# NVIDIA-Genomics-Research/DL4VC

Hardware: AMD Instinct MI355X
Metric: candidate-variants/sec (DAN fwd, 64 reads x 201 bp) (higher is better)
Workload: dtype f32

## Files before the change

dl4vc_amd/csrc/dan_device.h:

```cpp
#pragma once
#include "dan_kernels.h"

namespace dan {

typedef float v4f __attribute__((ext_vector_type(4)));

__device__ __forceinline__ v4f mfma16(float a, float b, v4f c) {
    return __builtin_amdgcn_mfma_f32_16x16x4f32(a, b, c, 0, 0, 0);
}

__device__ __forceinline__ v4f splat(float x) { return (v4f){x, x, x, x}; }

typedef const __attribute__((address_space(1))) v4f* gv4f_ptr;

__device__ __forceinline__ float relu1(float v) { return __builtin_amdgcn_fmed3f(v, 0.f, __builtin_inff()); }

__device__ __forceinline__ void gemm_tile(v4f (&acc)[NT], const v4f (&a)[NT], v4f& b, const float* next) {
#pragma unroll
    for (int s = 0; s < 4; ++s)
#pragma unroll
        for (int n = 0; n < NT; ++n) acc[n] = mfma16(a[n][s], b[s], acc[n]);
    b = *(const v4f*)next;
}

__device__ __forceinline__ void conv_gemm(v4f (&acc)[MTW][NT], const float* xs, gv4f_ptr wl, const v4f (&a_first)[NT],
                                          int kg, int ntaps, int dil, int lane, int m_base, int cnt) {
    const int pos = lane & 15, kk = lane >> 4;
    const int total = ntaps * kg;
    const int t0 = (ntaps == 3) ? -dil : 0;
    const float* xrow = xs + (HALO + m_base * 16 + pos) * LDS_S + kk * 4;
    const bool full = cnt == MTW;
    v4f a_nxt[NT], b[MTW];
#pragma unroll
    for (int n = 0; n < NT; ++n) a_nxt[n] = a_first[n];
    {
        const float* xb = xrow + t0 * LDS_S;
#pragma unroll
        for (int m = 0; m < MTW - 1; ++m) b[m] = *(const v4f*)(xb + m * 16 * LDS_S);
        b[MTW - 1] = full ? *(const v4f*)(xb + (MTW - 1) * 16 * LDS_S) : splat(0.f);
    }
    int t = 0, g = 0;
    for (int it = 0; it < total; ++it) {
        v4f a[NT];
#pragma unroll
        for (int n = 0; n < NT; ++n) a[n] = a_nxt[n];
        const int nx = (it + 1 < total) ? it + 1 : it;
#pragma unroll
        for (int n = 0; n < NT; ++n) a_nxt[n] = wl[(size_t)nx * (KGC * 64) + n * 64];
        int tn = t, gn = g + 1;
        if (gn == kg) { gn = 0; ++tn; }
        if (it + 1 == total) { tn = t; gn = g; }
        const float* xn = xrow + (t0 + tn * dil) * LDS_S + gn * 16;
#pragma unroll
        for (int m = 0; m < MTW - 1; ++m) gemm_tile(acc[m], a, b[m], xn + m * 16 * LDS_S);
        __builtin_amdgcn_sched_group_barrier(0x020, NT, 0);
#pragma unroll
        for (int m = 0; m < MTW - 1; ++m) {
            __builtin_amdgcn_sched_group_barrier(0x008, 4 * NT, 0);
            __builtin_amdgcn_sched_group_barrier(0x100, 1, 0);
        }
        if (full) gemm_tile(acc[MTW - 1], a, b[MTW - 1], xn + (MTW - 1) * 16 * LDS_S);
        t = tn; g = gn;
    }
}

template <int NW, bool RANGE = false, int TILES = MT>
__device__ __forceinline__ void bottleneck(const float* xs, const v4f (&wf)[KGC], const float* bbot, float* hrow, int L,
                                           int wave, int lane, int p_lo = 0) {
    constexpr int PSTEP = NW / 2;
    constexpr int NBT = (TILES + PSTEP - 1) / PSTEP;
    lane = (int)__builtin_amdgcn_mbcnt_hi(~0u, __builtin_amdgcn_mbcnt_lo(~0u, 0u));
    asm volatile("" : "+v"(lane));
    const int pos = lane & 15, kk = lane >> 4;
    const int n = wave & 1, p0 = wave >> 1;
    const float* xrow = xs + (HALO + pos) * LDS_S + kk * 4;
    int roff[NBT];
#pragma unroll
    for (int i = 0; i < NBT; ++i) roff[i] = min(p0 + PSTEP * i, TILES - 1) * 16 * LDS_S;
    v4f acc[NBT], b[NBT];
    {
        const v4f bias = *(const v4f*)(bbot + n * 16 + kk * 4);
#pragma unroll
        for (int i = 0; i < NBT; ++i) acc[i] = bias;
    }
#pragma unroll
    for (int i = 0; i < NBT; ++i) b[i] = *(const v4f*)(xrow + roff[i]);
#pragma unroll
    for (int g = 0; g < KGC; ++g) {
        const int gn = (g + 1 < KGC) ? g + 1 : g;
#pragma unroll
        for (int i = 0; i < NBT; ++i) {
#pragma unroll
            for (int s = 0; s < 4; ++s) acc[i] = mfma16(wf[g][s], b[i][s], acc[i]);
            b[i] = *(const v4f*)(xrow + roff[i] + gn * 16);
        }
#pragma unroll
        for (int i = 0; i < NBT; ++i) {
            __builtin_amdgcn_sched_group_barrier(0x008, 4, 0);
            __builtin_amdgcn_sched_group_barrier(0x100, 1, 0);
        }
    }
#pragma unroll
    for (int i = 0; i < NBT; ++i) {
        const int pt = p0 + PSTEP * i, p = pt * 16 + pos;
        if (pt < TILES && p < L && (!RANGE || p >= p_lo)) {
            v4f v = acc[i];
#pragma unroll
            for (int j = 0; j < 4; ++j) v[j] = relu1(v[j]);
            *(v4f*)((char*)hrow + (unsigned)(p * HPAD + n * 16 + kk * 4) * 4u) = v;
        }
    }
}

__device__ __forceinline__ void copy_out(const float* xs, float* dst, int lo, int hi, int tid) {
    for (int i = lo * (CPAD / 4) + tid; i < hi * (CPAD / 4); i += SEG_THREADS) {
        const int p = i >> 5, c4 = i & 31;
        ((v4f*)dst)[i] = *(const v4f*)(xs + (HALO + p) * LDS_S + c4 * 4);
    }
}

constexpr int MW = 7;
constexpr int WHB = 102;
constexpr int MW_SHORT = 6;
constexpr int WHB_SHORT = 94;
constexpr int MPOS_SHORT = WHB_SHORT + 16 * MW_SHORT;
constexpr int wino_half_base(int tw) { return tw == MW ? WHB : WHB_SHORT; }
constexpr int wino_cover(int tw) { return tw == MW ? MPOS : MPOS_SHORT; }
template <int TW = MW>
__device__ __forceinline__ int wino_base(int lane) {
    const int n = lane & 15;
    const int c = n & 1, hf = (n >> 2) & 1, q = ((n >> 1) & 1) + 2 * (((n >> 3) ^ (n >> 2)) & 1);
    return hf * wino_half_base(TW) + 4 * q * TW + c;
}

typedef float v2f __attribute__((ext_vector_type(2)));
__device__ __forceinline__ v4f pk_sub(v4f a, v4f b, v2f m1) {
    const v2f lo = __builtin_elementwise_fma((v2f){b[0], b[1]}, m1, (v2f){a[0], a[1]});
    const v2f hi = __builtin_elementwise_fma((v2f){b[2], b[3]}, m1, (v2f){a[2], a[3]});
    return (v4f){lo[0], lo[1], hi[0], hi[1]};
}
__device__ __forceinline__ v4f pk_add(v4f a, v4f b) { return a + b; }
template <int TW>
__device__ __forceinline__ void conv_gemm_wino(v4f (&acc)[TW][4], const float* xrow, gv4f_ptr wl, const v4f (&a_first)[4]) {
    v4f a_nxt[4];
#pragma unroll
    for (int k = 0; k < 4; ++k) a_nxt[k] = a_first[k];
    v4f xa = *(const v4f*)(xrow), xb = *(const v4f*)(xrow + 2 * LDS_S), xc = *(const v4f*)(xrow + 4 * LDS_S),
        xd = *(const v4f*)(xrow + 6 * LDS_S);
    float neg1 = -1.f;
    asm volatile("" : "+v"(neg1));
    const v2f m1 = {neg1, neg1};
    for (int g = 0; g < KGC; ++g) {
        v4f a[4];
#pragma unroll
        for (int k = 0; k < 4; ++k) a[k] = a_nxt[k];
        const int gn = (g + 1 < KGC) ? g + 1 : g;
#pragma unroll
        for (int k = 0; k < 4; ++k) a_nxt[k] = wl[(size_t)(k * KGC + gn) * (KGC * 64)];
        const float* xg = xrow + g * 16;
        const float* xn = xrow + gn * 16;
#pragma unroll
        for (int m = 0; m < TW; ++m) {
            v4f v[4];
            v[0] = pk_sub(xa, xc, m1); v[1] = pk_add(xb, xc); v[2] = pk_sub(xc, xb, m1); v[3] = pk_sub(xb, xd, m1);
            if (m + 1 < TW) {
                xa = xc; xb = xd;
                xc = *(const v4f*)(xg + (4 * m + 8) * LDS_S);
                xd = *(const v4f*)(xg + (4 * m + 10) * LDS_S);
            } else {
                xa = *(const v4f*)(xn); xb = *(const v4f*)(xn + 2 * LDS_S);
                xc = *(const v4f*)(xn + 4 * LDS_S); xd = *(const v4f*)(xn + 6 * LDS_S);
            }
            __builtin_amdgcn_s_setprio(3);
#pragma unroll
            for (int s = 0; s < 4; ++s)
#pragma unroll
                for (int k = 0; k < 4; ++k) acc[m][k] = mfma16(a[k][s], v[k][s], acc[m][k]);
            __builtin_amdgcn_s_setprio(0);
        }
    }
}

constexpr int WINO_ROWS_READ = HALO + WHB + 4 * (4 * MW - 1) + 1 + 4 + 1;

}
```

dl4vc_amd/csrc/dan_kernels.hip:

```cpp
#include "dan_device.h"

namespace dan {

#ifdef DAN_STAMPS
__device__ unsigned long long* g_stamps;
constexpr int NSTAMP = 64;
#define STAMP(k)                                                                                      \
    do {                                                                                              \
        __builtin_amdgcn_sched_barrier(0);                                                            \
        unsigned long long t_ = __builtin_amdgcn_s_memtime();                                         \
        __builtin_amdgcn_s_waitcnt(0xC07F);                                                           \
        if (lane == 0 && (k) < NSTAMP) g_stamps[((size_t)stamp_row * NWAVE + wave) * NSTAMP + (k)] = t_; \
        __builtin_amdgcn_sched_barrier(0);                                                            \
    } while (0)
#else
#define STAMP(k) do {} while (0)
#endif

static_assert((HALO + WHB + 4 * (4 * MW - 1) + 1 + 4 + 1) * LDS_S <= LDS_ROWS * LDS_S + MAX_LAYERS * CST_FLOATS, "wino reads stay inside LDS");
static_assert(WHB + 4 * (4 * MW - 1) + 3 >= MPOS - 1 && 4 * (4 * MW - 1) + 3 >= WHB - 1, "wino tiling covers the read");
static_assert(WHB_SHORT + 4 * (4 * MW_SHORT - 1) + 3 >= MPOS_SHORT - 1 && 4 * (4 * MW_SHORT - 1) + 3 >= WHB_SHORT - 1 && WHB_SHORT % 4 == 2,
              "short wino tiling covers its unit");

template <int TW>
__device__ __forceinline__ void gemm1x1_wino(v4f (&acc)[TW][2], const float* xrow, gv4f_ptr wl, v4f a_first) {
    v4f a_nxt = a_first, b[TW][2];
#pragma unroll
    for (int m = 0; m < TW; ++m)
#pragma unroll
        for (int o = 0; o < 2; ++o) b[m][o] = *(const v4f*)(xrow + (4 * m + 2 * o) * LDS_S);
    for (int g = 0; g < KGC; ++g) {
        const v4f a = a_nxt;
        const int gn = (g + 1 < KGC) ? g + 1 : g;
        a_nxt = wl[(size_t)gn * (KGC * 64)];
#pragma unroll
        for (int m = 0; m < TW; ++m) {
            __builtin_amdgcn_s_setprio(3);
#pragma unroll
            for (int s = 0; s < 4; ++s)
#pragma unroll
                for (int o = 0; o < 2; ++o) acc[m][o] = mfma16(a[s], b[m][o][s], acc[m][o]);
            __builtin_amdgcn_s_setprio(0);
#pragma unroll
            for (int o = 0; o < 2; ++o) b[m][o] = *(const v4f*)(xrow + (4 * m + 2 * o) * LDS_S + gn * 16);
        }
    }
}

template <bool WINO, bool PERSIST, bool SPLIT, int TW = MW, bool FOLD = false>
__global__ __launch_bounds__(SEG_THREADS, NWAVE / 4) void segment_kernel(SegmentArgs a_by_value) {
    static_assert(!FOLD || (PERSIST && !SPLIT), "the site-owning form is a persistent one-unit form");
    static_assert((!(SPLIT && WINO) && TW == MW) || (SPLIT && WINO && TW == MW_SHORT), "six tiles per lane: the split Winograd kernel, and only it");
    constexpr int TILES = TW == MW ? MT : (MPOS_SHORT + 15) / 16;
    __shared__ __attribute__((aligned(16))) float lds[LDS_ROWS * LDS_S + MAX_LAYERS * CST_FLOATS];
    float* const xs = lds;
    float* const cst = lds + LDS_ROWS * LDS_S;
    typedef const __attribute__((address_space(4))) SegmentArgs* kernarg_ptr;
    constexpr int UNITS = SPLIT ? 2 : 1;
    const int n_work = FOLD ? a_by_value.n_sites : (a_by_value.work_count ? *a_by_value.work_count : a_by_value.n_rows) * UNITS;
    const int per = FOLD ? a_by_value.xcd_sites : a_by_value.work_count ? (n_work + 7) >> 3 : a_by_value.xcd_rows * UNITS;
    const int xcd = blockIdx.x & 7;
    int j = blockIdx.x >> 3;
    int wk = xcd * per + j;
    if (j >= per || wk >= n_work) return;
    [[maybe_unused]] int fold_r = 0;
next_row:
    {
    kernarg_ptr ap = (kernarg_ptr)__builtin_amdgcn_kernarg_segment_ptr();
    if (PERSIST) asm volatile("" : "+s"(ap));
    auto args = [&]() -> decltype(auto) { if constexpr (PERSIST) return (*ap); else return (a_by_value); };
    const auto& a = args();
    [[maybe_unused]] const int unit = wk & 1;
    const int L = SPLIT ? (unit ? a.u_len[1] : a.u_len[0]) : a.L;
    const int Lw = SPLIT ? a.Lw : L;
    const int u_off = SPLIT ? (unit ? a.u_off[1] : a.u_off[0]) : 0;
    [[maybe_unused]] const int own_lo = SPLIT ? (unit ? a.own_lo[1] : a.own_lo[0]) : 0;
    [[maybe_unused]] const int own_hi = SPLIT ? (unit ? a.own_hi[1] : a.own_hi[0]) : L;
    [[maybe_unused]] const int stamp_row = wk;
    int tid = threadIdx.x;
    if (PERSIST) asm volatile("" : "+v"(tid));
    const int lane = tid & 63;
    const int wave = __builtin_amdgcn_readfirstlane(tid >> 6);
    const int wrow = SPLIT ? wk >> 1 : wk;
    const int row_index = FOLD ? wk * a.R + fold_r : __builtin_amdgcn_readfirstlane(a.work_count ? a.work[wrow] : wrow);
    const int site = FOLD ? wk : (int)((unsigned)row_index / (unsigned)a.R);
    const int r = FOLD ? fold_r : row_index - site * a.R;
    const size_t read_idx = (size_t)site * a.R + r;
    float* yrow = a.y + (read_idx * (size_t)Lw + u_off) * CPAD;
    float* yout = SPLIT ? a.y_out + (read_idx * (size_t)Lw + u_off) * CPAD : yrow;
    const int pos = lane & 15, kk = lane >> 4;
    const int cq = wave & 3, ph = wave >> 2;
    const int m_base = ph * MTW, cnt = ph ? MT - MTW : MTW;
    int chb[NT];
#pragma unroll
    for (int n = 0; n < NT; ++n) chb[n] = (cq * NT + n) * 16 + kk * 4;

    STAMP(0);
    [[maybe_unused]] const int wP0 = wino_base<TW>(lane);
    [[maybe_unused]] const int wlim = ((lane >> 2) & 1) ? wino_cover(TW) : wino_half_base(TW);
    [[maybe_unused]] const int chw = wave * 16 + kk * 4;
    auto dil_of = [&](int l) { return (l == 0) ? 1 : (l + 1 < a.n_layers ? a.dil_mid : a.dil_final); };
    auto wino_layer = [&](int l) { return WINO && l > 0; };
    constexpr bool CARRY = !(WINO && PERSIST);
    v4f pc0 = splat(0.f), pc1 = pc0, pc2 = pc0, pc3 = pc0, pn0 = pc0, pn1 = pc0, pn2 = pc0, pn3 = pc0;
    auto first_frags = [&](int l, v4f& f0, v4f& f1, v4f& f2, v4f& f3) {
        const float* blk = a.wl + (size_t)l * LAYER_STRIDE;
        if (wino_layer(l)) {
            gv4f_ptr w0 = (gv4f_ptr)(blk + WW_OFF) + wave * 64 + lane;
            constexpr size_t KS = (size_t)KGC * (KGC * 64);
            f0 = w0[0]; f1 = w0[KS]; f2 = w0[2 * KS]; f3 = w0[3 * KS];
        } else {
            gv4f_ptr w0 = (gv4f_ptr)(blk + W_OFF) + (cq * NT) * 64 + lane;
            f0 = w0[0]; f1 = w0[64];
        }
    };
    const bool l0_lookup = a.l_begin == 0 && a.l0_tab != nullptr && !(a.tap && a.tap_layer == 0) && (a.l_end - a.l_begin) <= L0_MAX_LAYERS;
    float* const tokf = cst + (a.l_end - a.l_begin) * CST_FLOATS;
    if ((!WINO || a.l_begin == 0) && !l0_lookup) first_frags(a.l_begin, pc0, pc1, pc2, pc3);
    auto stage_constants = [&]() {
        for (int i = tid; i < (a.l_end - a.l_begin) * CST_FLOATS; i += SEG_THREADS) {
            const int l = i / CST_FLOATS, j = i - l * CST_FLOATS;
            cst[i] = a.wl[(size_t)(a.l_begin + l) * LAYER_STRIDE + CST_OFF + j];
        }
    };

    if (a.l_begin == 0) {
        if (l0_lookup) {
            for (int i = tid; i < (LDS_ROWS - L) * (LDS_S / 4); i += SEG_THREADS) {
                const int rr = i / (LDS_S / 4), c4 = i - rr * (LDS_S / 4);
                const int row = rr < HALO ? rr : rr + L;
                *(v4f*)(xs + row * LDS_S + c4 * 4) = splat(0.f);
            }
        } else {
            for (int i = tid; i < LDS_ROWS * LDS_S / 4; i += SEG_THREADS) ((v4f*)xs)[i] = splat(0.f);
        }
        stage_constants();
        __syncthreads();
        const size_t rbase = read_idx * (size_t)Lw + u_off, sbase = (size_t)site * Lw + u_off;
        const int p = tid;
        const bool in = p < L;
        int tok = 0, q = 0, st = 0, rf = 0, rm = 0, vm = 0;
        if (in) {
            tok = a.reads[rbase + p]; q = a.qual[rbase + p]; st = a.strand[rbase + p];
            rf = a.ref[sbase + p]; rm = a.ref_mask[sbase + p]; vm = a.var_mask[sbase + p];
        }
        int tok_w = tok, rm_w = rm, vm_w = vm;
        if constexpr (SPLIT) {
            tok_w = rm_w = vm_w = 0;
            if (tid < Lw) { tok_w = a.reads[rbase - u_off + tid]; rm_w = a.ref_mask[sbase - u_off + tid]; vm_w = a.var_mask[sbase - u_off + tid]; }
        }
        const int agree_ref = __syncthreads_and((rm_w == 0) || (tok_w == rm_w));
        const int agree_var = __syncthreads_and((vm_w == 0) || (tok_w == vm_w));
        if (l0_lookup) {
            if (p <= L + 1) {
                const int pc = p - 1;
                int tk = 0, qq = 0, ss = 0, rr = 0, mm = 0, vv = 0;
                const bool inside = pc >= 0 && pc < L;
                if (inside) {
                    tk = a.reads[rbase + pc]; qq = a.qual[rbase + pc]; ss = a.strand[rbase + pc];
                    rr = a.ref[sbase + pc]; mm = a.ref_mask[sbase + pc]; vv = a.var_mask[sbase + pc];
                }
                float* t = tokf + p * L0_TOK;
                const v4f t0 = {__builtin_bit_cast(float, inside ? min(tk, VOCAB - 1) * 10 + min(rr, VOCAB - 1) : 100), (float)qq * 0.01f, (float)ss * 0.5f,
                                (inside && mm != 0) ? 1.f : 0.f};
                const v4f t1 = {(inside && vv != 0 && agree_var) ? 1.f : 0.f, (p == 0 && agree_ref) ? 1.f : 0.f, 0.f, 0.f};
                *(v4f*)t = t0; *(v4f*)(t + 4) = t1;
            }
        } else if (in) {
            float* row = xs + (HALO + p) * LDS_S;
            const float* er = a.emb + min(tok, VOCAB - 1) * EMBED;
            const float* ef = a.emb + min(rf, VOCAB - 1) * EMBED;
            const float* pp = a.pe + (u_off + p) * EMBED;
#pragma unroll
            for (int e = 0; e < EMBED; ++e) {
                const float pv = pp[e];
                row[e] = er[e] + pv;
                row[EMBED + e] = ef[e] + pv;
            }
            row[40] = (float)q * 0.01f;
            row[41] = (float)st * 0.5f;
            row[42] = (rm != 0 && agree_ref) ? 1.f : 0.f;
            row[43] = (vm != 0 && agree_var) ? 1.f : 0.f;
            row[44] = (rm != 0) ? 1.f : 0.f;
        }
    } else {
        const v4f* src = (const v4f*)yrow;
        const v4f* pl = a.pool ? (const v4f*)(a.pool + ((size_t)site * Lw + u_off) * CPAD) : nullptr;
        const int n4 = L * (CPAD / 4);
        constexpr int NP = TILES * 16 * (CPAD / 4) / SEG_THREADS;
        v4f vy[NP], vp[NP];
#pragma unroll
        for (int k = 0; k < NP; ++k) {
            const int i = tid + k * SEG_THREADS;
            vy[k] = (i < n4) ? src[i] : splat(0.f);
        }
        if (pl) {
#pragma unroll
            for (int k = 0; k < NP; ++k) {
                const int i = tid + k * SEG_THREADS;
                vp[k] = (i < n4) ? pl[i] : splat(0.f);
            }
        } else {
#pragma unroll
            for (int k = 0; k < NP; ++k) vp[k] = splat(0.f);
        }
        for (int i = tid; i < (LDS_ROWS - L) * (LDS_S / 4); i += SEG_THREADS) {
// ... 9 lines not shown
        }
        if (WINO && CARRY) first_frags(a.l_begin, pc0, pc1, pc2, pc3);
    }
    __syncthreads();
    STAMP(1);
    if (a.tap && a.tap_layer == 0 && a.l_begin == 0) copy_out(xs, a.tap + (read_idx * (size_t)Lw + u_off) * CPAD, own_lo, own_hi, tid);

    v4f wbot[KGC];
    auto layer_tail = [&](int l, const float* lc, bool late_prefetch) {
        [[maybe_unused]] const int sb = 2 + (l - a.l_begin) * 8;
        __syncthreads();
        STAMP(sb + 6);
        if (a.tap && a.tap_layer == l + 1) {
            int t = tid;
            asm volatile("" : "+v"(t));
            copy_out(xs, a.tap + (read_idx * (size_t)Lw + u_off) * CPAD, own_lo, own_hi, t);
        }
        if (WINO && CARRY && late_prefetch && l + 1 < a.l_end) first_frags(l + 1, pn0, pn1, pn2, pn3);
        if (!(FOLD && WINO) && a.has_hw && !(WINO && l + 1 < a.l_end) && !(FOLD && l + 1 == a.l_end))
            bottleneck<NWAVE, SPLIT, TILES>(xs, wbot, lc + CST_BBOT, a.h + (size_t)l * a.h_layer_stride + (read_idx * (size_t)Lw + u_off) * HPAD,
                                     own_hi, wave, lane, own_lo);
        STAMP(sb + 7);
        if (CARRY) { pc0 = pn0; pc1 = pn1; pc2 = pn2; pc3 = pn3; }
    };

    auto direct_layer = [&](int l) {
        const float* wblk = a.wl + (size_t)l * LAYER_STRIDE;
        const float* lc = cst + (l - a.l_begin) * CST_FLOATS;
        const bool residual = (a.res_mask >> l) & 1u;
        const int kg = (l == 0) ? KG0 : KGC;
        const int dil = dil_of(l);
        gv4f_ptr w_conv = (gv4f_ptr)(wblk + W_OFF) + (cq * NT) * 64 + lane;
        gv4f_ptr w_res = (gv4f_ptr)(wblk + WRES_OFF) + (cq * NT) * 64 + lane;
        gv4f_ptr w_bot = (gv4f_ptr)(wblk + WBOT_OFF) + lane;
        [[maybe_unused]] const int sb = 2 + (l - a.l_begin) * 8;
        if (!WINO && l + 1 < a.l_end) first_frags(l + 1, pn0, pn1, pn2, pn3);
        const bool from_global = (l == a.l_begin) && (a.l_begin != 0) && (a.pool != nullptr);
        v4f pre_res[NT];
#pragma unroll
        for (int n = 0; n < NT; ++n) pre_res[n] = residual ? w_res[n * 64] : splat(0.f);
        static_assert(NT == 2, "two direct-form fragments are carried");
        const v4f pre_dir[NT] = {pc0, pc1};

        v4f acc[MTW][NT];
        {
            v4f bias[NT];
#pragma unroll
            for (int n = 0; n < NT; ++n) bias[n] = *(const v4f*)(lc + CST_BIAS + chb[n]);
#pragma unroll
            for (int m = 0; m < MTW; ++m)
#pragma unroll
                for (int n = 0; n < NT; ++n) acc[m][n] = bias[n];
        }
        STAMP(sb + 0);
        conv_gemm(acc, xs, w_conv, pre_dir, kg, 3, dil, lane, m_base, cnt);
        STAMP(sb + 1);
        const bool bot_here = a.has_hw && !(WINO && l + 1 < a.l_end);
        if (bot_here && !residual) {
#pragma unroll
            for (int g = 0; g < KGC; ++g) wbot[g] = w_bot[(g * 2 + (wave & 1)) * 64];
        }
        {
            v4f sc[NT], sh[NT];
#pragma unroll
            for (int n = 0; n < NT; ++n) { sc[n] = *(const v4f*)(lc + CST_SCALE + chb[n]); sh[n] = *(const v4f*)(lc + CST_SHIFT + chb[n]); }
#pragma unroll
            for (int m = 0; m < MTW; ++m) {
                const bool live = ((m_base + m) * 16 + pos) < L;
#pragma unroll
                for (int n = 0; n < NT; ++n) {
                    v4f v = acc[m][n];
#pragma unroll
                    for (int j = 0; j < 4; ++j) v[j] = live ? relu1(v[j]) * sc[n][j] + sh[n][j] : 0.f;
                    acc[m][n] = v;
                }
            }
        }
        STAMP(sb + 2);
        __syncthreads();
        STAMP(sb + 3);
        if (residual) {
            v4f bres[NT];
#pragma unroll
            for (int n = 0; n < NT; ++n) bres[n] = *(const v4f*)(lc + CST_BRES + chb[n]);
            if (!from_global) {
#pragma unroll
                for (int m = 0; m < MTW; ++m) {
                    if (m < cnt) {
#pragma unroll
                        for (int n = 0; n < NT; ++n) {
                            v4f* cell = (v4f*)(xs + (HALO + (m_base + m) * 16 + pos) * LDS_S + chb[n]);
                            const v4f old = *cell;
                            *cell = acc[m][n];
                            acc[m][n] = old + bres[n];
                        }
                    }
                }
            } else {
#pragma unroll
                for (int m = 0; m < MTW; ++m) {
                    const int p = (m_base + m) * 16 + pos;
                    if (m < cnt) {
#pragma unroll
                        for (int n = 0; n < NT; ++n) {
                            const v4f old = (p < L) ? *(const v4f*)(yrow + (size_t)p * CPAD + chb[n]) : splat(0.f);
                            *(v4f*)(xs + (HALO + p) * LDS_S + chb[n]) = acc[m][n];
                            acc[m][n] = old + bres[n];
                        }
                    }
                }
            }
            __syncthreads();
            STAMP(sb + 4);
            conv_gemm(acc, xs, w_res, pre_res, KGC, 1, 0, lane, m_base, cnt);
            STAMP(sb + 5);
            if (bot_here) {
#pragma unroll
                for (int g = 0; g < KGC; ++g) wbot[g] = w_bot[(g * 2 + (wave & 1)) * 64];
            }
            __syncthreads();
#pragma unroll
            for (int m = 0; m < MTW; ++m) {
                const int p = (m_base + m) * 16 + pos;
                if (m < cnt) {
#pragma unroll
                    for (int n = 0; n < NT; ++n) *(v4f*)(xs + (HALO + p) * LDS_S + chb[n]) = (p < L) ? acc[m][n] : splat(0.f);
                }
            }
        } else {
#pragma unroll
            for (int m = 0; m < MTW; ++m) {
                if (m < cnt) {
#pragma unroll
                    for (int n = 0; n < NT; ++n)
                        *(v4f*)(xs + (HALO + (m_base + m) * 16 + pos) * LDS_S + chb[n]) = acc[m][n];
                }
            }
        }
        layer_tail(l, lc, true);
    };

    [[maybe_unused]] auto wino_layer_body = [&](int l) {
        if constexpr (WINO) {
        const float* wblk = a.wl + (size_t)l * LAYER_STRIDE;
        const float* lc = cst + (l - a.l_begin) * CST_FLOATS;
        const bool residual = (a.res_mask >> l) & 1u;
        gv4f_ptr w_bot = (gv4f_ptr)(wblk + WBOT_OFF) + lane;
        [[maybe_unused]] const int sb = 2 + (l - a.l_begin) * 8;
        const bool from_global = (l == a.l_begin) && (a.l_begin != 0) && (a.pool != nullptr);
        gv4f_ptr w_w = (gv4f_ptr)(wblk + WW_OFF) + wave * 64 + lane;
        gv4f_ptr w_r1 = (gv4f_ptr)(wblk + WRES_OFF) + wave * 64 + lane;
        float* xw = xs + (HALO + wP0) * LDS_S;
        v4f out[TW][2], pre_r1;
        int wp = wP0;
        float* xq;
        {
            v4f acc[TW][4];
            const v4f bias = *(const v4f*)(lc + CST_BIAS + chw);
#pragma unroll
            for (int m = 0; m < TW; ++m) { acc[m][0] = splat(0.f); acc[m][1] = bias; acc[m][2] = splat(0.f); acc[m][3] = splat(0.f); }
            STAMP(sb + 0);
            if constexpr (CARRY) {
                const v4f pre_w[4] = {pc0, pc1, pc2, pc3};
                conv_gemm_wino(acc, xw - 2 * LDS_S + kk * 4, w_w, pre_w);
            } else {
                gv4f_ptr w0 = w_w;
                const v4f pre_w[4] = {w0[0], w0[(size_t)KGC * (KGC * 64)], w0[(size_t)2 * KGC * (KGC * 64)], w0[(size_t)3 * KGC * (KGC * 64)]};
                conv_gemm_wino(acc, xw - 2 * LDS_S + kk * 4, w_w, pre_w);
            }
            STAMP(sb + 1);
            asm volatile("" : "+v"(wp));
            xq = xs + (HALO + wp) * LDS_S;
            const v4f sc = *(const v4f*)(lc + CST_SCALE + chw), sh = *(const v4f*)(lc + CST_SHIFT + chw);
            const v2f sc_lo = {sc[0], sc[1]}, sc_hi = {sc[2], sc[3]}, sh_lo = {sh[0], sh[1]}, sh_hi = {sh[2], sh[3]};
            auto half = [](v4f v, int h) { return (v2f){v[2 * h], v[2 * h + 1]}; };
            v2f neg1 = {-1.f, -1.f};
            asm volatile("" : "+v"(neg1));
            auto act = [](v2f y, v2f s, v2f t) {
                const v2f r = {relu1(y[0]), relu1(y[1])};
                return __builtin_elementwise_fma(r, s, t);
            };
#pragma unroll
            for (int m = 0; m < TW; ++m) {
                const v2f y0l = half(acc[m][0], 0) + half(acc[m][1], 0) + half(acc[m][2], 0), y0h = half(acc[m][0], 1) + half(acc[m][1], 1) + half(acc[m][2], 1);
                const v2f y1l = __builtin_elementwise_fma(half(acc[m][3], 0), neg1, __builtin_elementwise_fma(half(acc[m][2], 0), neg1, half(acc[m][1], 0)));
                const v2f y1h = __builtin_elementwise_fma(half(acc[m][3], 1), neg1, __builtin_elementwise_fma(half(acc[m][2], 1), neg1, half(acc[m][1], 1)));
                const v2f o0l = act(y0l, sc_lo, sh_lo), o0h = act(y0h, sc_hi, sh_hi), o1l = act(y1l, sc_lo, sh_lo), o1h = act(y1h, sc_hi, sh_hi);
                out[m][0] = (v4f){o0l[0], o0l[1], o0h[0], o0h[1]};
                out[m][1] = (v4f){o1l[0], o1l[1], o1h[0], o1h[1]};
            }
        }
        int wl = min(wlim, L);
        asm volatile("" : "+v"(wl));
        __builtin_amdgcn_sched_barrier(0);
        pre_r1 = residual ? w_r1[0] : splat(0.f);
        if (CARRY && !residual && l + 1 < a.l_end) first_frags(l + 1, pn0, pn1, pn2, pn3);
        if (a.has_hw && l > a.l_begin && wave < NWAVE / 2) {
            gv4f_ptr w_bp = (gv4f_ptr)(wblk - LAYER_STRIDE + WBOT_OFF) + lane;
#pragma unroll
            for (int g = 0; g < KGC; ++g) wbot[g] = w_bp[(g * 2 + (wave & 1)) * 64];
            bottleneck<NWAVE / 2, SPLIT, TILES>(xs, wbot, lc - CST_FLOATS + CST_BBOT,
                                         a.h + (size_t)(l - 1) * a.h_layer_stride + (read_idx * (size_t)Lw + u_off) * HPAD, own_hi, wave, lane, own_lo);
        }
        const bool bot_here = a.has_hw && !(l + 1 < a.l_end);
        if (bot_here && !residual) {
#pragma unroll
            for (int g = 0; g < KGC; ++g) wbot[g] = w_bot[(g * 2 + (wave & 1)) * 64];
        }
        STAMP(sb + 2);
        __syncthreads();
        STAMP(sb + 3);
        if (residual) {
            const v4f bres = *(const v4f*)(lc + CST_BRES + chw);
            if (from_global) {
#pragma unroll
                for (int m = 0; m < TW; ++m)
#pragma unroll
                    for (int o = 0; o < 2; ++o) {
                        const int p = wp + 4 * m + 2 * o;
                        if (p < wl) {
                            const v4f old = *(const v4f*)((const char*)yrow + (unsigned)(p * CPAD + chw) * 4u);
                            *(v4f*)(xq + (4 * m + 2 * o) * LDS_S + chw) = out[m][o];
                            out[m][o] = old + bres;
                        }
                    }
            } else {
#pragma unroll
                for (int m = 0; m < TW; ++m)
#pragma unroll
                    for (int o = 0; o < 2; ++o) {
                        const int p = wp + 4 * m + 2 * o;
                        if (p < wl) {
                            v4f* cell = (v4f*)(xq + (4 * m + 2 * o) * LDS_S + chw);
                            const v4f old = *cell;
                            *cell = out[m][o];
                            out[m][o] = old + bres;
                        }
                    }
            }
            __syncthreads();
            STAMP(sb + 4);
            gemm1x1_wino(out, xq + kk * 4, w_r1, pre_r1);
            STAMP(sb + 5);
            if (CARRY && l + 1 < a.l_end) first_frags(l + 1, pn0, pn1, pn2, pn3);
            if (bot_here) {
#pragma unroll
                for (int g = 0; g < KGC; ++g) wbot[g] = w_bot[(g * 2 + (wave & 1)) * 64];
            }
            __syncthreads();
#pragma unroll
            for (int m = 0; m < TW; ++m)
#pragma unroll
                for (int o = 0; o < 2; ++o) {
                    const int p = wp + 4 * m + 2 * o;
                    if (p < wl) *(v4f*)(xq + (4 * m + 2 * o) * LDS_S + chw) = out[m][o];
                }
        } else {
#pragma unroll
            for (int m = 0; m < TW; ++m)
#pragma unroll
                for (int o = 0; o < 2; ++o) {
                    const int p = wp + 4 * m + 2 * o;
                    if (p < wl) *(v4f*)(xq + (4 * m + 2 * o) * LDS_S + chw) = out[m][o];
                }
        }
        layer_tail(l, lc, false);
        }
    };

    auto lookup_layer0 = [&]() {
        const float* lc = cst;
        [[maybe_unused]] const int sb = 2;
        if (!WINO && 1 < a.l_end) first_frags(1, pn0, pn1, pn2, pn3);
        STAMP(sb + 0);
        const int c4 = tid & 31, pr = tid >> 5;
        const v4f bias = *(const v4f*)(lc + CST_BIAS + c4 * 4), sc = *(const v4f*)(lc + CST_SCALE + c4 * 4), sh = *(const v4f*)(lc + CST_SHIFT + c4 * 4);
        v4f wq[3], wst[3], wlen[3], wvar[3];
        {
            const float agree = tokf[5];
#pragma unroll
            for (int t = 0; t < 3; ++t) {
                auto wv = [&](int k) { return *(const v4f*)(a.l0_tab + L0_WSC_OFF + (k * 3 + t) * CPAD + c4 * 4); };
                wq[t] = wv(0); wst[t] = wv(1); wvar[t] = wv(3);
                wlen[t] = wv(4) + agree * wv(2);
            }
        }
        const v4f* tj = (const v4f*)(a.l0_tab + L0_TJ_OFF) + c4;
        const v4f* pe = (const v4f*)(a.l0_tab + L0_PE_OFF) + (size_t)u_off * (CPAD / 4) + c4;
#pragma unroll 4
        for (int k = 0; k < TILES; ++k) {
            const int p = min(pr + 16 * k, L - 1);
            const int var = (p == 0) ? 1 : (p == L - 1) ? 2 : 0;
            const v4f pe0 = pe[((size_t)var * Lw + p) * (CPAD / 4)];
            v4f s0[3], tv[3];
            v2f s1[3];
#pragma unroll
            for (int t = 0; t < 3; ++t) {
                s0[t] = *(const v4f*)(tokf + (p + t) * L0_TOK);
                s1[t] = *(const v2f*)(tokf + (p + t) * L0_TOK + 4);
            }
#pragma unroll
            for (int t = 0; t < 3; ++t) tv[t] = tj[(size_t)(t * L0_NTJ + __builtin_bit_cast(int, s0[t][0])) * (CPAD / 4)];
            v2f alo = {bias[0] + pe0[0], bias[1] + pe0[1]}, ahi = {bias[2] + pe0[2], bias[3] + pe0[3]};
            auto fma4 = [&](float sv, const v4f& w) {
                const v2f ss = {sv, sv};
                alo = __builtin_elementwise_fma(ss, (v2f){w[0], w[1]}, alo);
                ahi = __builtin_elementwise_fma(ss, (v2f){w[2], w[3]}, ahi);
            };
#pragma unroll
            for (int t = 0; t < 3; ++t) {
                alo += (v2f){tv[t][0], tv[t][1]}; ahi += (v2f){tv[t][2], tv[t][3]};
                fma4(s0[t][1], wq[t]);
                fma4(s0[t][2], wst[t]);
                fma4(s0[t][3], wlen[t]);
                fma4(s1[t][0], wvar[t]);
            }
            v4f v;
            v[0] = relu1(alo[0]) * sc[0] + sh[0]; v[1] = relu1(alo[1]) * sc[1] + sh[1];
            v[2] = relu1(ahi[0]) * sc[2] + sh[2]; v[3] = relu1(ahi[1]) * sc[3] + sh[3];
            *(v4f*)(xs + (HALO + p) * LDS_S + c4 * 4) = v;
        }
        STAMP(sb + 2);
        const bool bot_here = a.has_hw && !(WINO && 1 < a.l_end);
        if (bot_here) {
            gv4f_ptr w_bot = (gv4f_ptr)(a.wl + WBOT_OFF) + lane;
#pragma unroll
            for (int g = 0; g < KGC; ++g) wbot[g] = w_bot[(g * 2 + (wave & 1)) * 64];
        }
        layer_tail(0, lc, true);
    };

    if constexpr (WINO) {
        int l = a.l_begin;
        if (l == 0) { if (l0_lookup) lookup_layer0(); else direct_layer(0); l = 1; }
        for (; l < a.l_end; ++l) wino_layer_body(l);
    } else {
        int l = a.l_begin;
        if (l == 0 && l0_lookup) { lookup_layer0(); l = 1; }
        for (; l < a.l_end; ++l) direct_layer(l);
    }
    STAMP(62);
    if constexpr (FOLD) {
        const bool fin = a.fold_feat != nullptr;
        if (!fin) copy_out(xs, yout, own_lo, own_hi, tid);
        constexpr int NF = MT * 16 * (CPAD / 4) / SEG_THREADS;
        const int n4 = L * (CPAD / 4);
        v4f* sp = (v4f*)(a.fold_scratch + (size_t)blockIdx.x * (2 * (size_t)n4 * 4));
        int t = tid;
        asm volatile("" : "+v"(t));
        v4f fsum[NF], fmx[NF];
        if (r > 0) {
#pragma unroll
            for (int k = 0; k < NF; ++k) {
                const int i = t + k * SEG_THREADS;
                fsum[k] = (i < n4) ? sp[i] : splat(0.f);
            }
        } else {
#pragma unroll
            for (int k = 0; k < NF; ++k) fsum[k] = splat(0.f);
        }
        if (r > 0 && fin) {
#pragma unroll
            for (int k = 0; k < NF; ++k) {
                const int i = t + k * SEG_THREADS;
                fmx[k] = (i < n4) ? sp[n4 + i] : splat(0.f);
            }
        } else {
#pragma unroll
            for (int k = 0; k < NF; ++k) fmx[k] = splat(0.f);
        }
        if (a.has_hw) {
            const int ll = a.l_end - 1;
            bottleneck<NWAVE, false, TILES>(xs, wbot, cst + (ll - a.l_begin) * CST_FLOATS + CST_BBOT,
                                            a.h + (size_t)ll * a.h_layer_stride + read_idx * (size_t)Lw * HPAD, own_hi, wave, lane, own_lo);
        }
        const bool last_row = r + 1 == a.R;
#pragma unroll
        for (int k = 0; k < NF; ++k) {
            const int i = t + k * SEG_THREADS;
            const v4f v = (i < n4) ? *(const v4f*)(xs + (HALO + (i >> 5)) * LDS_S + (i & 31) * 4) : splat(0.f);
            v4f mx = v;
            if (r > 0) {
#pragma unroll
                for (int jj = 0; jj < 4; ++jj) mx[jj] = fmaxf(fmx[k][jj], v[jj]);
            }
            fmx[k] = mx;
            v4f sum = fsum[k];
            sum += v;
            fsum[k] = (fin && r == 0) ? v : sum;
        }
        if (!last_row) {
#pragma unroll
            for (int k = 0; k < NF; ++k) {
                const int i = t + k * SEG_THREADS;
                if (i < n4) sp[i] = fsum[k];
            }
            if (fin) {
#pragma unroll
                for (int k = 0; k < NF; ++k) {
                    const int i = t + k * SEG_THREADS;
                    if (i < n4) sp[n4 + i] = fmx[k];
                }
            }
        } else {
            const float fR = (float)a.R;
            __syncthreads();
            auto put = [&](const v4f (&src)[NF]) {
#pragma unroll
                for (int k = 0; k < NF; ++k) {
                    const int i = t + k * SEG_THREADS;
                    if (i < n4) *(v4f*)(xs + (HALO + (i >> 5)) * LDS_S + (i & 31) * 4) = src[k];
                }
            };
            if (!fin) {
                put(fsum);
                v4f* pl = (v4f*)(a.fold_pool + (size_t)site * n4 * 4);
#pragma unroll 1
                for (int i = t; i < n4; i += SEG_THREADS)
                    pl[i] = *(const v4f*)(xs + (HALO + (i >> 5)) * LDS_S + (i & 31) * 4) / splat(fR);
            } else {
                float* row = a.fold_feat + (size_t)site * a.fold_feat_stride;
                const int C = a.fold_C;
                put(fmx);
                __syncthreads();
#pragma unroll 1
                for (int c = wave; c < C; c += NWAVE)
#pragma unroll 1
                    for (int p = lane; p < L; p += 64) row[(unsigned)(c * L + p)] = xs[(HALO + p) * LDS_S + c];
                __syncthreads();
                put(fsum);
                __syncthreads();
                row += (size_t)C * L;
#pragma unroll 1
                for (int c = wave; c < C; c += NWAVE)
#pragma unroll 1
                    for (int p = lane; p < L; p += 64) row[(unsigned)(c * L + p)] = xs[(HALO + p) * LDS_S + c] / fR;
            }
        }
    } else {
        copy_out(xs, yout, own_lo, own_hi, tid);
    }
    STAMP(63);
    }
    if constexpr (FOLD) {
        if (++fold_r == a_by_value.R) {
            fold_r = 0;
            j += gridDim.x >> 3;
            wk = xcd * per + j;
        }
        __syncthreads();
        if (j < per && wk < n_work) goto next_row;
    } else if constexpr (PERSIST) {
        j += gridDim.x >> 3;
        wk = xcd * per + j;
        __syncthreads();
        if (j < per && wk < n_work) goto next_row;
    }
}

int segment_fold_workgroups(int n_sites, int max_wgs) {
    const int w = max_wgs & ~7, need = 8 * ((n_sites + 7) / 8);
    return w < need ? w : need;
}

void launch_segment(const SegmentArgs& a0, int n_sites, int max_wgs, hipStream_t s) {
    SegmentArgs a = a0;
    a.n_rows = n_sites * a.R;
    a.xcd_rows = ((n_sites + 7) / 8) * a.R;
    const bool split = a.units == 2;
    if (!split) { a.units = 1; a.Lw = a.L; a.y_out = a.y; }
    const int units = split ? 2 : 1;
    if (a.fold) {
        a.n_sites = n_sites;
        a.xcd_sites = (n_sites + 7) / 8;
        const dim3 grid((unsigned)segment_fold_workgroups(n_sites, max_wgs)), blk(SEG_THREADS);
        if (a.wino) hipLaunchKernelGGL((segment_kernel<true, true, false, MW, true>), grid, blk, 0, s, a);
        else hipLaunchKernelGGL((segment_kernel<false, true, false, MW, true>), grid, blk, 0, s, a);
        return;
    }
    const bool persist = a.work_count != nullptr && max_wgs >= 8 && max_wgs < a.n_rows * units;
    const dim3 grid((unsigned)(persist ? (max_wgs & ~7) : 8 * a.xcd_rows * units)), blk(SEG_THREADS);
    if (split) {
        static_assert((304 + 1) / 2 + 1 + 2 * (MAX_LAYERS - 1) <= MPOS_SHORT, "a split Winograd unit fits the six-tile form");
        const bool wino = a.wino && a.L <= MPOS_SHORT;
        a.wino = wino;
        if (persist) {
            if (wino) hipLaunchKernelGGL((segment_kernel<true, true, true, MW_SHORT>), grid, blk, 0, s, a);
            else hipLaunchKernelGGL((segment_kernel<false, true, true>), grid, blk, 0, s, a);
        } else {
            if (wino) hipLaunchKernelGGL((segment_kernel<true, false, true, MW_SHORT>), grid, blk, 0, s, a);
            else hipLaunchKernelGGL((segment_kernel<false, false, true>), grid, blk, 0, s, a);
        }
    } else if (persist) {
        if (a.wino) hipLaunchKernelGGL((segment_kernel<true, true, false>), grid, blk, 0, s, a);
        else hipLaunchKernelGGL((segment_kernel<false, true, false>), grid, blk, 0, s, a);
    } else {
        if (a.wino) hipLaunchKernelGGL((segment_kernel<true, false, false>), grid, blk, 0, s, a);
        else hipLaunchKernelGGL((segment_kernel<false, false, false>), grid, blk, 0, s, a);
    }
}

__global__ __launch_bounds__(256) void row_map_kernel(const uint8_t* __restrict__ reads, const uint8_t* __restrict__ qual,
                                                      const uint8_t* __restrict__ strand, int* __restrict__ row_src, int R, int L) {
    __shared__ int empty[1024];
    const int site = blockIdx.x, tid = threadIdx.x, lane = tid & 63, wave = tid >> 6;
    for (int r = wave; r < R; r += 4) {
        const size_t base = ((size_t)site * R + r) * L;
        unsigned any = 0;
        for (int p = lane; p < L; p += 64) any |= (unsigned)reads[base + p] | (unsigned)qual[base + p] | (unsigned)strand[base + p];
        const bool none = __ballot(any != 0) == 0ull;
        if (lane == 0 && r < 1024) empty[r] = none;
    }
    __syncthreads();
    int first = -1;
    for (int r = 0; r < R && r < 1024; ++r)
        if (empty[r]) { first = r; break; }
    for (int r = tid; r < R; r += 256) row_src[(size_t)site * R + r] = site * R + ((r < 1024 && empty[r]) ? first : r);
}

__global__ __launch_bounds__(1024) void work_list_kernel(const int* __restrict__ row_src, int* __restrict__ work,
                                                         int* __restrict__ count, int n_sites, int R) {
    __shared__ int offs[4096 + 1];
    const int tid = threadIdx.x;
    int total = 0;
    for (int base = 0; base < n_sites; base += 4096) {
        const int n = min(4096, n_sites - base);
        for (int sidx = tid; sidx < n; sidx += 1024) {
            int c = 0;
            const int* rs = row_src + (size_t)(base + sidx) * R;
            for (int r = 0; r < R; ++r) c += rs[r] == (base + sidx) * R + r;
            offs[sidx + 1] = c;
        }
        __syncthreads();
        if (tid == 0) {
            offs[0] = total;
            for (int i = 0; i < n; ++i) offs[i + 1] += offs[i];
        }
        __syncthreads();
        for (int sidx = tid; sidx < n; sidx += 1024) {
            int o = offs[sidx];
            const int* rs = row_src + (size_t)(base + sidx) * R;
            for (int r = 0; r < R; ++r)
                if (rs[r] == (base + sidx) * R + r) work[o++] = (base + sidx) * R + r;
        }
        total = offs[n];
        __syncthreads();
    }
    if (tid == 0) *count = total;
}

void launch_row_map(const uint8_t* reads, const uint8_t* qual, const uint8_t* strand, int* row_src, int* work, int* count,
                    int n_sites, int R, int L, hipStream_t s) {
    hipLaunchKernelGGL(row_map_kernel, dim3(n_sites), dim3(256), 0, s, reads, qual, strand, row_src, R, L);
    hipLaunchKernelGGL(work_list_kernel, dim3(1), dim3(1024), 0, s, row_src, work, count, n_sites, R);
}

__global__ __launch_bounds__(256) void read_mean_kernel(const v4f* __restrict__ y, v4f* __restrict__ pool, int R, int L,
                                                        const int* __restrict__ row_src) {
    const int n4 = L * (CPAD / 4);
    const int i = blockIdx.x * 256 + threadIdx.x;
    if (i >= n4) return;
    const int site = blockIdx.y;
    v4f sum = splat(0.f);
    if (row_src) {
        const int* rs = row_src + (size_t)site * R;
#pragma unroll 8
        for (int r = 0; r < R; ++r) sum += y[(size_t)rs[r] * n4 + i];
    } else {
        const v4f* src = y + (size_t)site * R * n4 + i;
#pragma unroll 8
        for (int r = 0; r < R; ++r) sum += src[(size_t)r * n4];
    }
    pool[(size_t)site * n4 + i] = sum / splat((float)R);
}

void launch_read_mean(const float* y, float* pool, int n_sites, int R, int L, const int* row_src, hipStream_t s) {
    const int n4 = L * (CPAD / 4);
    hipLaunchKernelGGL(read_mean_kernel, dim3((n4 + 255) / 256, n_sites), dim3(256), 0, s, (const v4f*)y, (v4f*)pool, R, L,
                       row_src);
}

__global__ __launch_bounds__(256) void final_pool_kernel(const v4f* __restrict__ y, float* __restrict__ feat,
                                                         long long fs, int R, int L, int C, const int* __restrict__ row_src) {
    constexpr int PT = 32, PS = PT + 1;
    __shared__ float tmax[CPAD * PS], tavg[CPAD * PS];
    const int pt = blockIdx.x, site = blockIdx.y, tid = threadIdx.x;
    const int c4 = tid & 31, pl = tid >> 5;
    const int n4 = L * (CPAD / 4);
#pragma unroll
    for (int half = 0; half < PT / 8; ++half) {
        const int pp = half * 8 + pl, p = pt * PT + pp;
        v4f mx = splat(0.f), av = splat(0.f);
        if (p < L) {
            const size_t off = (size_t)p * (CPAD / 4) + c4;
            const int* rs = row_src ? row_src + (size_t)site * R : nullptr;
            auto row = [&](int r) { return rs ? y[(size_t)rs[r] * n4 + off] : y[((size_t)site * R + r) * n4 + off]; };
            mx = row(0);
            v4f sum = mx;
#pragma unroll 8
            for (int r = 1; r < R; ++r) {
                const v4f v = row(r);
#pragma unroll
                for (int j = 0; j < 4; ++j) mx[j] = fmaxf(mx[j], v[j]);
                sum += v;
            }
            av = sum / splat((float)R);
        }
#pragma unroll
        for (int j = 0; j < 4; ++j) {
            tmax[(c4 * 4 + j) * PS + pp] = mx[j];
            tavg[(c4 * 4 + j) * PS + pp] = av[j];
        }
    }
    __syncthreads();
    float* row = feat + (size_t)site * fs;
    for (int idx = tid; idx < CPAD * PT; idx += 256) {
        const int c = idx / PT, pp = idx % PT, p = pt * PT + pp;
        if (c < C && p < L) {
            row[(size_t)c * L + p] = tmax[c * PS + pp];
            row[(size_t)C * L + (size_t)c * L + p] = tavg[c * PS + pp];
        }
    }
}

void launch_final_pool(const float* y, float* feat, long long fs, int n_sites, int R, int L, int C, const int* row_src,
                       hipStream_t s) {
    hipLaunchKernelGGL(final_pool_kernel, dim3((L + 31) / 32, n_sites), dim3(256), 0, s, (const v4f*)y, feat, fs, R, L, C,
                       row_src);
}

constexpr int HW_DH = 16;
__global__ __launch_bounds__(512) void highway_kernel(const float* __restrict__ h, long long hls,
                                                      const v4f* __restrict__ wc, long long wcls,
                                                      const float* __restrict__ bc, float* __restrict__ feat,
                                                      long long fs, int feat_off, int n_rows, int R, int L, int H,
                                                      const int* __restrict__ row_src) {
    __shared__ __attribute__((aligned(16))) char ring[2][8][4][1024];
    const int tid = threadIdx.x, lane = tid & 63, wave = tid >> 6;
    const int r16 = lane & 15, kk = lane >> 4;
    const int layer = blockIdx.y;
    const int row0 = blockIdx.x * 128 + wave * 16;
    const size_t K = (size_t)L * HPAD;
    const int row = min(row0 + r16, n_rows - 1);
    const float* arow = h + (size_t)layer * hls + (size_t)(row_src ? row_src[row] : row) * K + kk * 4;
    const v4f* wl = wc + (size_t)layer * wcls + lane;
    v4f acc0 = splat(0.f), acc1 = splat(0.f);
    const int n_ph = (L + 7) >> 3;
    v4f ar[HW_DH][2];
#pragma unroll
    for (int d = 0; d < HW_DH; ++d) {
// ... 241 lines not shown
```

Before: 14030.

## Use six Winograd tiles plus a plain remainder tile for reads just over coverage

For one-unit reads up to 206 positions (L=201 falls here), the Winograd conv path now walks six tiles per lane. A 16-position remainder tile is handled by direct 3-tap MFMAs interleaved into the Winograd loop and the 1x1 residual GEMM, instead of walking seven tiles. Reads that fit within six tiles use the six-tile form with no remainder. This is meant to cut the padded MFMA work and LDS reads of the seventh tile. In exchange it adds extra weight loads, register pressure and another kernel instantiation.

```diff
diff --git a/dl4vc_amd/csrc/dan_device.h b/dl4vc_amd/csrc/dan_device.h
--- a/dl4vc_amd/csrc/dan_device.h
+++ b/dl4vc_amd/csrc/dan_device.h
@@ -140,8 +140,10 @@
     return (v4f){lo[0], lo[1], hi[0], hi[1]};
 }
 __device__ __forceinline__ v4f pk_add(v4f a, v4f b) { return a + b; }
-template <int TW>
-__device__ __forceinline__ void conv_gemm_wino(v4f (&acc)[TW][4], const float* xrow, gv4f_ptr wl, const v4f (&a_first)[4]) {
+template <int TW, bool REM = false>
+__device__ __forceinline__ void conv_gemm_wino(v4f (&acc)[TW][4], const float* xrow, gv4f_ptr wl, const v4f (&a_first)[4],
+                                               [[maybe_unused]] v4f& racc, [[maybe_unused]] const float* xr, [[maybe_unused]] gv4f_ptr wd) {
+    static_assert(!REM || TW == 6, "the remainder tile's taps follow tiles 1, 3 and 5 of a six-tile walk");
     v4f a_nxt[4];
 #pragma unroll
     for (int k = 0; k < 4; ++k) a_nxt[k] = a_first[k];
@@ -157,6 +159,11 @@
         const int gn = (g + 1 < KGC) ? g + 1 : g;
 #pragma unroll
         for (int k = 0; k < 4; ++k) a_nxt[k] = wl[(size_t)(k * KGC + gn) * (KGC * 64)];
+        [[maybe_unused]] v4f ra[3], rb;
+        if constexpr (REM) {
+#pragma unroll
+            for (int t = 0; t < 3; ++t) ra[t] = wd[(size_t)(t * KGC + g) * (KGC * 64)];
+        }
         const float* xg = xrow + g * 16;
         const float* xn = xrow + gn * 16;
 #pragma unroll
@@ -171,15 +178,29 @@
                 xa = *(const v4f*)(xn); xb = *(const v4f*)(xn + 2 * LDS_S);
                 xc = *(const v4f*)(xn + 4 * LDS_S); xd = *(const v4f*)(xn + 6 * LDS_S);
             }
+            if constexpr (REM) {
+                if ((m & 1) == 0) rb = *(const v4f*)(xr + (m >> 1) * 2 * LDS_S + g * 16);
+            }
             __builtin_amdgcn_s_setprio(3);
 #pragma unroll
             for (int s = 0; s < 4; ++s)
 #pragma unroll
                 for (int k = 0; k < 4; ++k) acc[m][k] = mfma16(a[k][s], v[k][s], acc[m][k]);
+            if constexpr (REM) {
+                if (m & 1) {
+#pragma unroll
+                    for (int s = 0; s < 4; ++s) racc = mfma16(ra[m >> 1][s], rb[s], racc);
+                }
+            }
             __builtin_amdgcn_s_setprio(0);
         }
     }
 }
+template <int TW>
+__device__ __forceinline__ void conv_gemm_wino(v4f (&acc)[TW][4], const float* xrow, gv4f_ptr wl, const v4f (&a_first)[4]) {
+    v4f none = splat(0.f);
+    conv_gemm_wino<TW, false>(acc, xrow, wl, a_first, none, nullptr, nullptr);
+}
 
 constexpr int WINO_ROWS_READ = HALO + WHB + 4 * (4 * MW - 1) + 1 + 4 + 1;
 
diff --git a/dl4vc_amd/csrc/dan_kernels.hip b/dl4vc_amd/csrc/dan_kernels.hip
--- a/dl4vc_amd/csrc/dan_kernels.hip
+++ b/dl4vc_amd/csrc/dan_kernels.hip
@@ -19,12 +19,16 @@
 
 static_assert((HALO + WHB + 4 * (4 * MW - 1) + 1 + 4 + 1) * LDS_S <= LDS_ROWS * LDS_S + MAX_LAYERS * CST_FLOATS, "wino reads stay inside LDS");
 static_assert(WHB + 4 * (4 * MW - 1) + 3 >= MPOS - 1 && 4 * (4 * MW - 1) + 3 >= WHB - 1, "wino tiling covers the read");
+static_assert(HALO + MPOS_SHORT + 15 + 2 < LDS_ROWS && MPOS_SHORT + 16 <= MPOS, "the remainder tile's taps stay inside the image");
 static_assert(WHB_SHORT + 4 * (4 * MW_SHORT - 1) + 3 >= MPOS_SHORT - 1 && 4 * (4 * MW_SHORT - 1) + 3 >= WHB_SHORT - 1 && WHB_SHORT % 4 == 2,
               "short wino tiling covers its unit");
 
-template <int TW>
-__device__ __forceinline__ void gemm1x1_wino(v4f (&acc)[TW][2], const float* xrow, gv4f_ptr wl, v4f a_first) {
+template <int TW, bool REM = false>
+__device__ __forceinline__ void gemm1x1_wino(v4f (&acc)[TW][2], const float* xrow, gv4f_ptr wl, v4f a_first,
+                                             [[maybe_unused]] v4f& racc, [[maybe_unused]] const float* xr) {
     v4f a_nxt = a_first, b[TW][2];
+    [[maybe_unused]] v4f rb;
+    if constexpr (REM) rb = *(const v4f*)xr;
 #pragma unroll
     for (int m = 0; m < TW; ++m)
 #pragma unroll
@@ -40,18 +44,28 @@
             for (int s = 0; s < 4; ++s)
 #pragma unroll
                 for (int o = 0; o < 2; ++o) acc[m][o] = mfma16(a[s], b[m][o][s], acc[m][o]);
+            if constexpr (REM) {
+                if (m + 1 == TW) {
+#pragma unroll
+                    for (int s = 0; s < 4; ++s) racc = mfma16(a[s], rb[s], racc);
+                }
+            }
             __builtin_amdgcn_s_setprio(0);
 #pragma unroll
             for (int o = 0; o < 2; ++o) b[m][o] = *(const v4f*)(xrow + (4 * m + 2 * o) * LDS_S + gn * 16);
-        }
-    }
-}
-
-template <bool WINO, bool PERSIST, bool SPLIT, int TW = MW, bool FOLD = false>
+            if constexpr (REM) {
+                if (m + 1 == TW) rb = *(const v4f*)(xr + gn * 16);
+            }
+        }
+    }
+}
+
+template <bool WINO, bool PERSIST, bool SPLIT, int TW = MW, bool FOLD = false, bool REM = false>
 __global__ __launch_bounds__(SEG_THREADS, NWAVE / 4) void segment_kernel(SegmentArgs a_by_value) {
     static_assert(!FOLD || (PERSIST && !SPLIT), "the site-owning form is a persistent one-unit form");
-    static_assert((!(SPLIT && WINO) && TW == MW) || (SPLIT && WINO && TW == MW_SHORT), "six tiles per lane: the split Winograd kernel, and only it");
-    constexpr int TILES = TW == MW ? MT : (MPOS_SHORT + 15) / 16;
+    static_assert(TW == MW ? !(SPLIT && WINO) : (WINO && TW == MW_SHORT), "six tiles per lane: Winograd forms only, and the split one always");
+    static_assert(!REM || (WINO && !SPLIT && TW == MW_SHORT), "the remainder tile [190, 206): beside six Winograd tiles of a one-unit read");
+    constexpr int TILES = (SPLIT && WINO) ? (MPOS_SHORT + 15) / 16 : MT;
     __shared__ __attribute__((aligned(16))) float lds[LDS_ROWS * LDS_S + MAX_LAYERS * CST_FLOATS];
     float* const xs = lds;
     float* const cst = lds + LDS_ROWS * LDS_S;
@@ -367,6 +381,8 @@
         gv4f_ptr w_r1 = (gv4f_ptr)(wblk + WRES_OFF) + wave * 64 + lane;
         float* xw = xs + (HALO + wP0) * LDS_S;
         v4f out[TW][2], pre_r1;
+        [[maybe_unused]] v4f rout = splat(0.f);
+        [[maybe_unused]] int rp = MPOS_SHORT + pos;
         int wp = wP0;
         float* xq;
         {
@@ -374,17 +390,25 @@
             const v4f bias = *(const v4f*)(lc + CST_BIAS + chw);
 #pragma unroll
             for (int m = 0; m < TW; ++m) { acc[m][0] = splat(0.f); acc[m][1] = bias; acc[m][2] = splat(0.f); acc[m][3] = splat(0.f); }
+            if constexpr (REM) rout = bias;
             STAMP(sb + 0);
+            auto gemm = [&](const v4f (&pre_w)[4]) {
+                if constexpr (REM)
+                    conv_gemm_wino<TW, true>(acc, xw - 2 * LDS_S + kk * 4, w_w, pre_w, rout, xs + (HALO + rp - 2) * LDS_S + kk * 4, (gv4f_ptr)(wblk + W_OFF) + wave * 64 + lane);
+                else
+                    conv_gemm_wino(acc, xw - 2 * LDS_S + kk * 4, w_w, pre_w);
+            };
             if constexpr (CARRY) {
                 const v4f pre_w[4] = {pc0, pc1, pc2, pc3};
-                conv_gemm_wino(acc, xw - 2 * LDS_S + kk * 4, w_w, pre_w);
+                gemm(pre_w);
             } else {
                 gv4f_ptr w0 = w_w;
                 const v4f pre_w[4] = {w0[0], w0[(size_t)KGC * (KGC * 64)], w0[(size_t)2 * KGC * (KGC * 64)], w0[(size_t)3 * KGC * (KGC * 64)]};
-                conv_gemm_wino(acc, xw - 2 * LDS_S + kk * 4, w_w, pre_w);
+                gemm(pre_w);
             }
             STAMP(sb + 1);
             asm volatile("" : "+v"(wp));
+            if constexpr (REM) asm volatile("" : "+v"(rp));
             xq = xs + (HALO + wp) * LDS_S;
             const v4f sc = *(const v4f*)(lc + CST_SCALE + chw), sh = *(const v4f*)(lc + CST_SHIFT + chw);
             const v2f sc_lo = {sc[0], sc[1]}, sc_hi = {sc[2], sc[3]}, sh_lo = {sh[0], sh[1]}, sh_hi = {sh[2], sh[3]};
@@ -404,7 +428,12 @@
                 out[m][0] = (v4f){o0l[0], o0l[1], o0h[0], o0h[1]};
                 out[m][1] = (v4f){o1l[0], o1l[1], o1h[0], o1h[1]};
             }
-        }
+            if constexpr (REM) {
+                const v2f rl = act(half(rout, 0), sc_lo, sh_lo), rh = act(half(rout, 1), sc_hi, sh_hi);
+                rout = (v4f){rl[0], rl[1], rh[0], rh[1]};
+            }
+        }
+        [[maybe_unused]] float* const rcell = xs + (HALO + rp) * LDS_S + chw;
         int wl = min(wlim, L);
         asm volatile("" : "+v"(wl));
         __builtin_amdgcn_sched_barrier(0);
@@ -439,6 +468,13 @@
                             out[m][o] = old + bres;
                         }
                     }
+                if constexpr (REM) {
+                    if (rp < L) {
+                        const v4f old = *(const v4f*)((const char*)yrow + (unsigned)(rp * CPAD + chw) * 4u);
+                        *(v4f*)rcell = rout;
+                        rout = old + bres;
+                    }
+                }
             } else {
 #pragma unroll
                 for (int m = 0; m < TW; ++m)
@@ -452,10 +488,17 @@
                             out[m][o] = old + bres;
                         }
                     }
+                if constexpr (REM) {
+                    if (rp < L) {
+                        const v4f old = *(const v4f*)rcell;
+                        *(v4f*)rcell = rout;
+                        rout = old + bres;
+                    }
+                }
             }
             __syncthreads();
             STAMP(sb + 4);
-            gemm1x1_wino(out, xq + kk * 4, w_r1, pre_r1);
+            gemm1x1_wino<TW, REM>(out, xq + kk * 4, w_r1, pre_r1, rout, xs + (HALO + rp) * LDS_S + kk * 4);
             STAMP(sb + 5);
             if (CARRY && l + 1 < a.l_end) first_frags(l + 1, pn0, pn1, pn2, pn3);
             if (bot_here) {
@@ -470,6 +513,9 @@
                     const int p = wp + 4 * m + 2 * o;
                     if (p < wl) *(v4f*)(xq + (4 * m + 2 * o) * LDS_S + chw) = out[m][o];
                 }
+            if constexpr (REM) {
+                if (rp < L) *(v4f*)rcell = rout;
+            }
         } else {
 #pragma unroll
             for (int m = 0; m < TW; ++m)
@@ -478,6 +524,9 @@
                     const int p = wp + 4 * m + 2 * o;
                     if (p < wl) *(v4f*)(xq + (4 * m + 2 * o) * LDS_S + chw) = out[m][o];
                 }
+            if constexpr (REM) {
+                if (rp < L) *(v4f*)rcell = rout;
+            }
         }
         layer_tail(l, lc, false);
         }
@@ -685,11 +734,14 @@
     const bool split = a.units == 2;
     if (!split) { a.units = 1; a.Lw = a.L; a.y_out = a.y; }
     const int units = split ? 2 : 1;
+    const bool six = !split && a.L <= MPOS_SHORT, rem = !split && !six && a.L <= MPOS_SHORT + 16;
     if (a.fold) {
         a.n_sites = n_sites;
         a.xcd_sites = (n_sites + 7) / 8;
         const dim3 grid((unsigned)segment_fold_workgroups(n_sites, max_wgs)), blk(SEG_THREADS);
-        if (a.wino) hipLaunchKernelGGL((segment_kernel<true, true, false, MW, true>), grid, blk, 0, s, a);
+        if (a.wino && rem) hipLaunchKernelGGL((segment_kernel<true, true, false, MW_SHORT, true, true>), grid, blk, 0, s, a);
+        else if (a.wino && six) hipLaunchKernelGGL((segment_kernel<true, true, false, MW_SHORT, true>), grid, blk, 0, s, a);
+        else if (a.wino) hipLaunchKernelGGL((segment_kernel<true, true, false, MW, true>), grid, blk, 0, s, a);
         else hipLaunchKernelGGL((segment_kernel<false, true, false, MW, true>), grid, blk, 0, s, a);
         return;
     }
@@ -707,10 +759,14 @@
             else hipLaunchKernelGGL((segment_kernel<false, false, true>), grid, blk, 0, s, a);
         }
     } else if (persist) {
-        if (a.wino) hipLaunchKernelGGL((segment_kernel<true, true, false>), grid, blk, 0, s, a);
+        if (a.wino && rem) hipLaunchKernelGGL((segment_kernel<true, true, false, MW_SHORT, false, true>), grid, blk, 0, s, a);
+        else if (a.wino && six) hipLaunchKernelGGL((segment_kernel<true, true, false, MW_SHORT>), grid, blk, 0, s, a);
+        else if (a.wino) hipLaunchKernelGGL((segment_kernel<true, true, false>), grid, blk, 0, s, a);
         else hipLaunchKernelGGL((segment_kernel<false, true, false>), grid, blk, 0, s, a);
     } else {
-        if (a.wino) hipLaunchKernelGGL((segment_kernel<true, false, false>), grid, blk, 0, s, a);
+        if (a.wino && rem) hipLaunchKernelGGL((segment_kernel<true, false, false, MW_SHORT, false, true>), grid, blk, 0, s, a);
+        else if (a.wino && six) hipLaunchKernelGGL((segment_kernel<true, false, false, MW_SHORT>), grid, blk, 0, s, a);
+        else if (a.wino) hipLaunchKernelGGL((segment_kernel<true, false, false>), grid, blk, 0, s, a);
         else hipLaunchKernelGGL((segment_kernel<false, false, false>), grid, blk, 0, s, a);
     }
 }
```

Result: faster. 14250 (median of 6 runs) (+1.5%).
